# rrahn/libspm

Measured on AMD Instinct MI355X. Metric: Gbases/s scanned, Myers k<=3 |P|=100, higher is better.
Workload: dtype u32

## Files before the change

include/spm_hip.h:

```cpp
#ifndef SPM_HIP_H
#define SPM_HIP_H

#include <stddef.h>
#include <stdint.h>

#ifdef __cplusplus
extern "C" {
#endif

typedef struct spm_ctx spm_ctx;
typedef struct spm_text spm_text;
typedef struct spm_patterns spm_patterns;
typedef struct spm_hits spm_hits;
typedef struct spm_jst spm_jst;
typedef struct spm_jst_hits spm_jst_hits;

enum spm_status {
    SPM_OK = 0,
    SPM_E_INVALID = -1,
    SPM_E_HIP = -2,
    SPM_E_NOMEM = -3,
    SPM_E_UNSUPPORTED = -4,
    SPM_E_OVERFLOW = -5,
    SPM_E_PEER = -6
// ... 77 lines not shown
uint32_t spm_hip_patterns_count(const spm_patterns *p);
int spm_hip_patterns_needle(const spm_patterns *p, uint32_t pattern, uint8_t *out, uint32_t cap, uint32_t *len);

typedef struct spm_build_stats {
    float ms_total;
    float ms_tables;
    float ms_index;
    float ms_upload;
    uint32_t threads;
    uint32_t passes;
    uint32_t dense;
    uint32_t anchor_sixteenths;
    uint64_t keys;
    uint32_t stride, key_len;
    uint64_t bytes_device;
} spm_build_stats;
int spm_hip_patterns_build_stats(const spm_patterns *p, spm_build_stats *out);

size_t spm_hip_patterns_state_stride(const spm_patterns *p);
int spm_hip_patterns_state_init(const spm_patterns *p, void *state);

int spm_hip_scan(spm_ctx *ctx, const spm_text *text, uint64_t begin, uint64_t end, const spm_patterns *patterns,
                 const spm_scan_opts *opts, const void *state_in, void *state_out, spm_hits **out);

int spm_hip_scan_segments(spm_ctx *ctx, const spm_text *text, const uint64_t *seg_offsets, uint64_t n_segments,
                          const spm_patterns *patterns, const spm_scan_opts *opts, spm_hits **out);

int spm_hip_hits_view(spm_hits *hits, const spm_hit **records, uint64_t *n);
int spm_hip_hits_device(spm_hits *hits, const void **device_records, uint64_t *n);
int spm_hip_hits_copy_device(spm_hits *hits, void *device_dst, uint64_t cap, uint64_t *n);
// ... 668 lines not shown
```

libspm_amd/capi.py:

```python
from __future__ import annotations

import ctypes as C
import os
import subprocess

_PKG = os.path.dirname(os.path.abspath(__file__))
SO_PATH = os.path.join(_PKG, "libspm_hip.so")
CSRC = os.path.join(_PKG, "csrc")

ALGO_SHIFTOR, ALGO_MYERS, ALGO_MYERS_PREFIX, ALGO_HORSPOOL = 0, 1, 2, 3
ENGINE_AUTO, ENGINE_BRUTE, ENGINE_FILTER = 0, 1, 2
SCAN_IGNORE_PACKED = 1
SCAN_DEFER = 2
SCAN_ALIGNABLE = 4
MAX_NEEDLE = 2048


class SpmError(RuntimeError):
    pass


class Hit(C.Structure):
    _fields_ = [("pos", C.c_uint64), ("pattern", C.c_uint32), ("score", C.c_int32)]

# ... 28 lines not shown

class BuildStats(C.Structure):
    _fields_ = [
        ("ms_total", C.c_float),
        ("ms_tables", C.c_float),
        ("ms_index", C.c_float),
        ("ms_upload", C.c_float),
        ("threads", C.c_uint32),
        ("passes", C.c_uint32),
        ("dense", C.c_uint32),
        ("anchor_sixteenths", C.c_uint32),
        ("keys", C.c_uint64),
        ("stride", C.c_uint32),
        ("key_len", C.c_uint32),
        ("bytes_device", C.c_uint64),
    ]


class JstAllele(C.Structure):
    _fields_ = [("pos", C.c_uint64), ("ref_len", C.c_uint32), ("alt_len", C.c_uint32), ("alt_off", C.c_uint64)]


class JstHit(C.Structure):
    _fields_ = [("pos", C.c_uint64), ("haplotype", C.c_uint32), ("pattern", C.c_uint32), ("score", C.c_int32),
                ("reserved", C.c_uint32)]


class JstStats(C.Structure):
    _fields_ = [
        ("haplotype_symbols", C.c_uint64),
# ... 593 lines not shown
```

libspm_amd/csrc/filter_dense.hip:

```cpp
#include "filter_launch.hpp"
#include "filter_dense.hpp"

filter_kernel select_dense_kernel(const filter_index &F, bool km)
{
    if (F.dense) {
        switch (F.n_pat) {
        case 0:
        case 1: return seed_filter_dense_kernel<4, 1>;
        case 2: return seed_filter_dense_kernel<4, 2>;
        case 3: return seed_filter_dense_kernel<4, 3>;
        default: return nullptr;
        }
    }
    if (F.hash_variant == 4) {
        if (F.stride == 1)
            return km ? seed_filter_dense_kernel<4, 1, 1, true> : seed_filter_dense_kernel<4, 1, 1, false>;
        if (F.stride == 2)
            return km ? seed_filter_dense_kernel<4, 1, 2, true> : seed_filter_dense_kernel<4, 1, 2, false>;
    }
    return nullptr;
}

void warm_dense_kernels()
{
// ... 4 lines not shown
```

libspm_amd/csrc/filter_dense.hpp:

```cpp
#pragma once

#include "filter_stream.hpp"

namespace spm_hip
{

constexpr uint32_t kDenseQueueCap = 192;
constexpr int kDenseBatches = 3;

template <int NP>
__device__ __forceinline__ uint32_t dense_select(const filter_params &P, uint32_t w, uint32_t prev)
{
    const uint32_t X = alignbit(w, prev, 2);
    const uint32_t Y = alignbit(w, prev, 4);
    uint32_t sel = 0;
#pragma unroll
    for (int i = 0; i < NP; ++i) {
        const uint32_t C0 = (P.pat_c[i] & 3u) * 0x55555555u, M0 = (P.pat_cm[i] & 3u) * 0x55555555u;
        const uint32_t C1 = (P.pat_c[i] >> 2) * 0x55555555u, M1 = (P.pat_cm[i] >> 2) * 0x55555555u;
        uint32_t t = ((X ^ C0) & M0) | ((Y ^ C1) & M1);
        t |= t >> 1;
        sel |= ~t;
    }
    return sel & 0x55555555u;
}

struct dense_queue
{
    uint32_t key[kDenseQueueCap];
    uint32_t off[kDenseQueueCap];
};
static_assert(sizeof(dense_queue) == kDenseQueueBytes, "filter_params.hpp sizes the launch's LDS");

__device__ __forceinline__ void dense_drain(const filter_params &P, dense_queue &Q, uint32_t &qn, bool all, uint64_t span_base,
                                            uint32_t lane, const uint32_t *lds)
{
    while (qn >= 64 || (all && qn != 0)) {
// ... 25 lines not shown
            const uint32_t x0 = bk[b].x ^ f2, x1 = bk[b].y ^ f2, x2 = bk[b].z ^ f2, x3 = bk[b].w ^ f2;
            const uint32_t z = ((x0 - 0x00010001u) & ~x0) | ((x1 - 0x00010001u) & ~x1) | ((x2 - 0x00010001u) & ~x2) |
                               ((x3 - 0x00010001u) & ~x3);
            const bool hit = v[b] && ((z & 0x80008000u) != 0 || (bk[b].w >> 16) == kDenseAcceptAll);
            if (__ballot(hit) != 0) {
                if (__builtin_amdgcn_readfirstlane(cand_chunk_of(P, lds)[5]) == 0) {
                    const int64_t ts = (int64_t)span_base + (int64_t)off[b] - 16;
                    const bool has = hit && ts >= (int64_t)P.lo && (uint64_t)ts + P.key_len <= P.hi;
                    emit_survivors(P, has, key[b], has ? (uint64_t)ts : 0, lane, lds);
                }
            }
        }
    }
}

template <int UU, int NP, int S, bool KM>
__device__ __forceinline__ void dense_group(const filter_params &P, const uint4 (&cur)[UU], uint64_t gbase, uint64_t span_base,
                                            uint32_t &carry_in, uint32_t lane, const uint32_t *lds, dense_queue &Q, uint32_t &qn)
{
    static_assert(UU % 2 == 0 || UU == 1, "words are taken in pairs");
    uint32_t w[UU], prev[UU];
#pragma unroll
    for (int u = 0; u < UU; ++u)
        pack_with_prev(cur[u], lane, carry_in, w[u], prev[u]);
    const uint32_t goff = (uint32_t)(gbase - span_base) + lane * 16;
#pragma unroll
    for (int j = 0; j < UU; j += 2) {
        constexpr bool pair = UU > 1;
        const uint32_t w0 = w[j], p0 = prev[j], w1 = w[pair ? j + 1 : j], p1 = prev[pair ? j + 1 : j];
        const uint32_t kmask = KM ? P.key_mask : 0xFFFFFFFFu;
        static_assert(kDenseBloomBits == 20, "the word address below takes bits 5..19 of the index");
        uint32_t pm = 0;
        if constexpr (S == 0) {
            uint32_t todo = dense_select<NP>(P, w0, p0);
            if (pair)
                todo |= dense_select<NP>(P, w1, p1) << 1;
            while (todo != 0) {
                const uint32_t b = (uint32_t)__ffs(todo) - 1u;
                todo &= todo - 1;
                const bool odd = (b & 1u) != 0;
                const uint64_t both = ((uint64_t)(odd ? w1 : w0) << 32) | (odd ? p1 : p0);
                const uint32_t key = (uint32_t)(both >> ((b & ~1u) + 2u));
                const uint32_t h = key ^ (key >> 13);
                const uint32_t word = *reinterpret_cast<const uint32_t *>(reinterpret_cast<const uint8_t *>(lds) + ((h >> 3) & 0x1FFFCu));
                pm |= __builtin_amdgcn_ubfe(word, h, 1) << b;
            }
        } else {
#pragma unroll
            for (int u = 0; u < (pair ? 2 : 1); ++u) {
#pragma unroll
                for (int d = S; d <= 16; d += S) {
// ... 14 lines not shown
            const uint32_t key = (uint32_t)(both >> ((b & ~1u) + 2u)) & kmask;
            const uint64_t mm = __ballot(pos);
            if (pos) {
                const uint32_t q = qn + __popcll(mm & ((1ull << lane) - 1));
                Q.key[q] = key;
                Q.off[q] = goff + (uint32_t)j * 1024u + (odd ? 1024u : 0u) + (b >> 1) + 1u;
            }
            qn += __popcll(mm);
            queue_sync();
            if (qn > kDenseQueueCap - 64)
                dense_drain(P, Q, qn, false, span_base, lane, lds);
        }
    }
}

template <int U, int NP, int S = 0, bool KM = false>
__global__ __launch_bounds__(1024) void seed_filter_dense_kernel(const filter_params P)
{
    extern __shared__ uint32_t lds[];
    stream_stage(P, lds);

    const uint32_t lane = threadIdx.x & 63;
    const uint32_t waves_per_wg = blockDim.x >> 6;
    const uint32_t wave_in_wg = (uint32_t)__builtin_amdgcn_readfirstlane(threadIdx.x >> 6);
    dense_queue &Q = *reinterpret_cast<dense_queue *>(lds + P.lds_words + kCandLdsSlot + kCandRec * 16 +
                                                      (sizeof(dense_queue) / 4) * wave_in_wg);
    uint32_t qn = 0;

    const stream_geometry G = stream_geometry_of(P.lo, P.hi, 1024, P.span_chunks);
    const uint64_t span = P.span_chunks;
    const uint8_t *lane_text = P.text + G.base0 + (uint64_t)lane * 16;
// ... 18 lines not shown
#pragma unroll
            for (int u = 0; u < U; ++u)
                nxt[u] = load16_stream(lane_text + (ch + u) * 1024);
            for (; ch < fast_end; ch += U) {
                uint4 cur[U];
#pragma unroll
                for (int u = 0; u < U; ++u)
                    cur[u] = nxt[u];
                const bool more = ch + U < fast_end;
                const uint64_t pf = more ? ch + U : ch;
                const uint64_t ustride = more ? 1024 : 0;
#pragma unroll
                for (int u = 0; u < U; ++u)
                    nxt[u] = load16_stream(lane_text + pf * 1024 + (uint64_t)u * ustride);
                __builtin_amdgcn_sched_barrier(0);
                dense_group<U, NP, S, KM>(P, cur, G.base0 + ch * 1024, span_base, carry_in, lane, lds, Q, qn);
            }
        }
        for (; ch < c_end; ++ch) {
            uint4 one[1];
            one[0] = load_text16(P.text, G.base0 + ch * 1024 + (uint64_t)lane * 16, P.hi);
            dense_group<1, NP, S, KM>(P, one, G.base0 + ch * 1024, span_base, carry_in, lane, lds, Q, qn);
        }
        dense_drain(P, Q, qn, true, span_base, lane, lds);
    }
    surv_close(P, cand_chunk_of(P, lds), lane);
}

}
```

libspm_amd/csrc/filter_shared.hpp:

```cpp
#pragma once

#include "hd.hpp"

namespace spm_hip
{

constexpr uint32_t kKeyMax = 16;
constexpr uint32_t kKeyMin = 9;
constexpr double kMaxSurvivorShare = 0.08;

constexpr uint32_t kMergeMinK = 8;
struct seed_plan
{
    uint32_t n, q;
};
SPM_HD inline seed_plan plan_seeds(uint32_t m, uint32_t k)
{
    const uint32_t surplus = (k >= kMergeMinK && k <= 1000 && m / (k + 2) >= kKeyMin) ? 2u : 1u;
    return {k + surplus, m / (k + surplus)};
}

constexpr uint32_t kBloomProbes = 4;

SPM_HD inline uint32_t bloom_hash(uint32_t key, uint32_t i)
// ... 34 lines not shown
    return x ^ (x >> 16);
}

constexpr uint32_t kDensePatterns = 3;
constexpr uint32_t kDenseBloomBits = 20;
constexpr uint32_t kDenseSlots = 8;
constexpr uint32_t kDenseAcceptAll = 0x7FFFu;

SPM_HD inline uint32_t dense_bloom_index(uint32_t key)
{
    return (key ^ (key >> 13)) & ((1u << kDenseBloomBits) - 1);
}
SPM_HD inline uint32_t dense_bucket(uint32_t key, uint32_t bucket_shift) { return (key * 0x9E3779B1u) >> bucket_shift; }
SPM_HD inline uint32_t dense_fp(uint32_t key) { return 0x8000u | ((key ^ (key >> 15) ^ (key >> 23)) & 0x7FFFu); }

SPM_HD inline bool dense_anchored(uint32_t d, const uint32_t *c, const uint32_t *cm, uint32_t n_pat)
{
    for (uint32_t i = 0; i < n_pat; ++i)
        if (((d ^ c[i]) & cm[i]) == 0)
            return true;
    return false;
}

constexpr uint32_t kRngRun = 0x8000u;
constexpr uint32_t kRngSingle = 0x2000u;
constexpr uint32_t kRngWhole = 0x1000u;
constexpr uint32_t kSeedChecked = 0x4000u;

}
```

libspm_amd/csrc/index_dense.hpp:

```cpp
#pragma once

#include <chrono>
#include <cstdio>

#include "index_tables.hpp"

namespace spm_hip
{

struct dense_anchor_set
{
    uint32_t n_pat = 0, c[kDensePatterns] = {0, 0, 0}, cm[kDensePatterns] = {0, 0, 0};
    uint32_t dimers = 0;
    uint32_t sixteenths() const { return (uint32_t)__builtin_popcount(dimers); }
};

inline dense_anchor_set anchor_union(const dense_anchor_set &a, uint32_t c, uint32_t cm)
{
    dense_anchor_set r = a;
    r.c[r.n_pat] = c & cm;
    r.cm[r.n_pat] = cm;
    ++r.n_pat;
    r.dimers |= dimer_mask_of(c, cm);
    return r;
}

inline uint32_t dense_pick(const uint8_t *pat, uint32_t m, uint32_t dimers, uint32_t c, uint32_t want, uint16_t *pos)
{
    if (m < kKeyMax)
        return 0;
    uint32_t n = 0;
    for (uint32_t i = 0; i + kKeyMax <= m && n < want; ++i) {
        if (!((dimers >> dimer_at(pat, i)) & 1u))
            continue;
        if (n >= c && i < (uint32_t)pos[n - c] + kKeyMax)
            continue;
        pos[n++] = (uint16_t)i;
    }
    return n;
}

constexpr uint32_t kDenseCmax = 4;

inline uint32_t dense_layout(const uint8_t *pat, uint32_t m, uint32_t k, uint32_t dimers, uint16_t *pos, uint32_t &n_out)
{
    for (uint32_t c = 1; c <= kDenseCmax; ++c) {
        const uint32_t want = c * k + 1;
        if (want > 255)
            break;
        if (dense_pick(pat, m, dimers, c, want, pos) == want) {
            n_out = want;
            return c;
        }
    }
    return 0;
}

constexpr uint32_t kDenseMaxPieces = kDenseCmax * 7 + 1;

inline bool dense_eligible(const needle_view &nv)
{
    if (nv.sigma != 4 || nv.max_k >= kMergeMinK || nv.n == 0)
        return false;
    for (uint32_t p = 0; p < nv.n; ++p) {
        const uint32_t m = (uint32_t)nv.m[p];
        if (m < kKeyMax * (nv.errors(p) + 1) || m > 2047)
            return false;
    }
    return true;
}

inline uint64_t dense_uncovered(const needle_view &nv, uint32_t dimers, size_t begin, size_t end, size_t step,
                                std::vector<uint32_t> *list = nullptr, size_t cap = 0)
{
    uint64_t bad = 0;
    uint16_t pos[kDenseMaxPieces];
    for (size_t p = begin; p < end; p += step) {
        uint32_t n = 0;
        if (dense_layout(nv.needle(p), (uint32_t)nv.m[p], nv.errors(p), dimers, pos, n) == 0) {
            ++bad;
            if (list && list->size() < cap)
                list->push_back((uint32_t)p);
        }
    }
    return bad;
}

struct anchor_search
{
    const needle_view &nv;
    unsigned nt;
    size_t sample_step;
    std::vector<uint32_t> hard;
};

inline uint64_t uncovered_all(anchor_search &S, uint32_t dimers)
{
    std::vector<uint64_t> part(S.nt, 0);
    std::vector<std::vector<uint32_t>> lists(S.nt);
    parallel_slices(S.nv.n, S.nt,
                    [&](size_t b, size_t e, unsigned t) { part[t] = dense_uncovered(S.nv, dimers, b, e, 1, &lists[t], 8); });
    uint64_t s = 0;
    for (unsigned t = 0; t < S.nt; ++t) {
        s += part[t];
        for (uint32_t p : lists[t])
            if (S.hard.size() < 256)
                S.hard.push_back(p);
    }
    return s;
}

inline bool try_rung(anchor_search &S, const std::vector<dense_anchor_set> &cands, dense_anchor_set &best_seen)
{
    const needle_view &nv = S.nv;
    std::vector<uint64_t> base(cands.size(), 0);
    parallel_slices(cands.size(), S.nt, [&](size_t b, size_t e, unsigned) {
        for (size_t i = b; i < e; ++i)
            base[i] = dense_uncovered(nv, cands[i].dimers, 0, nv.n, S.sample_step);
    });
    std::vector<uint8_t> tried(cands.size(), 0);
    uint64_t best_fail = ~0ull;
    for (int attempt = 0; attempt < 4; ++attempt) {
        size_t best = cands.size();
        uint64_t best_bad = ~0ull;
        for (size_t i = 0; i < cands.size(); ++i) {
            if (tried[i])
                continue;
            uint64_t bad = base[i];
            for (uint32_t p : S.hard)
                bad += 4096 * dense_uncovered(nv, cands[i].dimers, p, (size_t)p + 1, 1);
            if (bad < best_bad) {
                best_bad = bad;
                best = i;
            }
        }
        if (best == cands.size())
            break;
        tried[best] = 1;
        const size_t hard_before = S.hard.size();
        const uint64_t fail = uncovered_all(S, cands[best].dimers);
        if (fail < best_fail) {
            best_fail = fail;
            best_seen = cands[best];
        }
        if (fail == 0)
            return true;
        if (S.hard.size() == hard_before || fail > nv.n / 2000 + 4)
            break;
        uint64_t placed = 0, asked = 0;
        for (size_t h = hard_before; h < S.hard.size(); ++h)
            for (size_t i = 0; i < cands.size(); i += 3) {
                ++asked;
                placed += dense_uncovered(nv, cands[i].dimers, S.hard[h], (size_t)S.hard[h] + 1, 1) == 0 ? 1 : 0;
            }
        if (2 * placed > asked)
            break;
    }
    return false;
}

inline std::vector<dense_anchor_set> anchor_extensions(const dense_anchor_set &base, uint32_t care)
{
    std::vector<dense_anchor_set> r;
    for (uint32_t cm = 0; cm < 16; ++cm) {
        if ((uint32_t)__builtin_popcount(cm) != care)
            continue;
        for (uint32_t c = 0; c < 16; ++c)
            if ((c & ~cm) == 0 && (dimer_mask_of(c, cm) & base.dimers) == 0)
                r.push_back(anchor_union(base, c, cm));
    }
    return r;
}

struct anchor_rung
{
    int extends;
    uint32_t care;
    bool dimer_pairs;
};
constexpr anchor_rung kAnchorLadder[] = {
    {-1, 3, true},
    {0, 4, false},
    {-1, 2, false},
    {2, 4, false},
    {2, 3, false},
    {-1, 1, false},
    {5, 2, false},
    {-1, 0, false},
};
constexpr size_t kAnchorRungs = sizeof(kAnchorLadder) / sizeof(kAnchorLadder[0]);

inline std::vector<dense_anchor_set> rung_candidates(const anchor_rung &R, const dense_anchor_set *best_of_rung)
{
    const dense_anchor_set none;
    std::vector<dense_anchor_set> c = anchor_extensions(R.extends < 0 ? none : best_of_rung[R.extends], R.care);
    if (R.dimer_pairs)
        for (uint32_t d0 = 0; d0 < 16; ++d0)
            for (uint32_t d1 = d0 + 1; d1 < 16; ++d1)
                if (__builtin_popcount(d0 ^ d1) != 1)
                    c.push_back(anchor_union(anchor_union(none, d0, 15), d1, 15));
    return c;
}

inline bool choose_dense_anchors(const needle_view &nv, const index_tuning &T, dense_anchor_set &out)
{
    anchor_search S{nv, T.n_threads(), std::max<size_t>(1, nv.n / 1024), {}};
    const int max_density = T.dense >= 2 ? 16 : 8;
    dense_anchor_set best_of_rung[kAnchorRungs];
    for (size_t rung = 0; rung < kAnchorRungs; ++rung) {
        const std::vector<dense_anchor_set> c = rung_candidates(kAnchorLadder[rung], best_of_rung);
        if (c.empty() || (int)c[0].sixteenths() < T.dense_min_density)
            continue;
        if ((int)c[0].sixteenths() > max_density)
            return false;
        if (try_rung(S, c, best_of_rung[rung])) {
            out = best_of_rung[rung];
            return true;
        }
    }
    return false;
}

struct dense_layouts
{
    std::vector<uint8_t> c, n;
    std::vector<uint32_t> first;
    std::vector<uint16_t> pos;
};

inline dense_layouts dense_first_fit(const needle_view &nv, unsigned nt, uint32_t dimers)
{
    dense_layouts L;
    L.c.assign(nv.n, 0);
    L.n.assign(nv.n, 0);
    L.first.assign(nv.n + 1, 0);
    std::vector<std::vector<uint16_t>> pos_of(nt);
    parallel_slices(nv.n, nt, [&](size_t b, size_t e, unsigned t) {
        uint16_t pos[kDenseMaxPieces];
        std::vector<uint16_t> &out = pos_of[t];
        out.reserve((e - b) * 5);
        for (size_t p = b; p < e; ++p) {
            uint32_t n = 0;
            L.c[p] = (uint8_t)dense_layout(nv.needle(p), (uint32_t)nv.m[p], nv.errors(p), dimers, pos, n);
            L.n[p] = (uint8_t)n;
            out.insert(out.end(), pos, pos + n);
        }
    });
    for (uint32_t p = 0; p < nv.n; ++p)
        L.first[p + 1] = L.first[p] + L.n[p];
    L.pos.reserve(L.first[nv.n]);
    for (unsigned t = 0; t < nt; ++t)
        L.pos.insert(L.pos.end(), pos_of[t].begin(), pos_of[t].end());
    return L;
}

inline void dense_share_bits(const needle_view &nv, const index_tuning &T, uint32_t dimers, const std::vector<uint8_t> &cc,
                             const std::vector<uint32_t> &first, std::vector<uint16_t> &pos_flat)
{
    thread_team team(T.n_threads());
    std::vector<uint16_t> ref(1u << kDenseBloomBits, 0);
    std::vector<uint8_t> placed(nv.n, 0);
    std::vector<uint32_t> bit_of(pos_flat.size(), 0), fresh_bit(pos_flat.size(), 0);
    for (uint32_t p = 0; p < nv.n; ++p)
        if (cc[p] != 1) {
            for (uint32_t s = first[p]; s < first[p + 1]; ++s)
                ++ref[bit_of[s] = dense_bloom_index(window_key(4, nv.needle(p), pos_flat[s], kKeyMax))];
            placed[p] = 1;
        }
    constexpr uint32_t kRounds = 24;
    std::vector<uint16_t> fresh(pos_flat.size());
    const unsigned nt = team.size();
// ... 14 lines not shown
                    const uint32_t need = first[p + 1] - first[p];
                    if (cc[p] != 1 || need == 0)
                        continue;
                    const uint8_t *pat = nv.needle(p);
                    const uint32_t m = (uint32_t)nv.m[p];
                    uint32_t own[kDenseMaxPieces];
                    for (uint32_t j = 0; j < need; ++j)
                        own[j] = placed[p] ? bit_of[first[p] + j] : 0xFFFFFFFFu;
                    cpos.clear();
                    cbit.clear();
                    shared.clear();
                    uint32_t key = window_key(4, pat, 0, kKeyMax);
                    for (uint32_t i = 0; i + kKeyMax <= m; ++i) {
                        if (i)
                            key = (key >> 2) | ((uint32_t)(pat[i + kKeyMax - 1] & 3u) << 30);
                        if (!((dimers >> (key & 15u)) & 1u))
                            continue;
                        const uint32_t bit = dense_bloom_index(key);
                        uint32_t mine = 0;
                        for (uint32_t j = 0; j < need; ++j)
                            mine += own[j] == bit ? 1u : 0u;
                        cpos.push_back((uint16_t)i);
                        cbit.push_back(bit);
                        shared.push_back(ref[bit] > mine ? 1 : 0);
                    }
                    const uint32_t nc = (uint32_t)cpos.size();
                    nxt.assign(nc + 1, nc);
                    for (uint32_t i = 0, t = 0; i < nc; ++i) {
                        while (t < nc && cpos[t] < cpos[i] + kKeyMax)
                            ++t;
                        nxt[i] = t;
// ... 84 lines not shown
    });
    return keys;
}

inline filter_index dense_pass_header(const dense_anchor_set &A, size_t n_keys)
{
    filter_index F;
    F.dense = 1;
    F.key_len = kKeyMax;
    F.stride = 1;
    F.n_pat = A.n_pat;
    for (uint32_t i = 0; i < A.n_pat; ++i) {
        F.pat_c[i] = A.c[i];
        F.pat_cm[i] = A.cm[i];
    }
    F.dimer_set = A.dimers;
    F.n_keys = n_keys;
    F.n_entries = n_keys;
    F.hash_variant = 3;
    return F;
}

inline int build_dense_index(const needle_view &nv, const index_tuning &T, seed_index &X)
{
    using iclk = std::chrono::steady_clock;
    auto ms = [&](iclk::time_point a) { return std::chrono::duration<double, std::milli>(iclk::now() - a).count(); };
    const unsigned nt = T.n_threads();
    const auto t0 = iclk::now();
    dense_anchor_set A;
    if (!choose_dense_anchors(nv, T, A))
        return SPM_OK;
    const double ms_anchors = ms(t0);
    const auto t1 = iclk::now();
    dense_layouts L = dense_first_fit(nv, nt, A.dimers);
    const double ms_first_fit = ms(t1);
    dense_share_bits(nv, T, A.dimers, L.c, L.first, L.pos);
    const double ms_share = ms(t1) - ms_first_fit;
    std::vector<index_kv> keys = dense_pieces(nv, nt, L, X);
    const double ms_layout = ms(t1);
    const auto t2 = iclk::now();
    filter_index F = dense_pass_header(A, keys.size());
    build_bits_level1(keys, F);
    const double ms_level1 = ms(t2);
    const auto t3 = iclk::now();
    build_directory(keys, F, X.h_entries);
    if (trace_on()) {
        uint64_t set = 0;
        for (uint32_t w : F.h_image)
            set += (uint64_t)__builtin_popcount(w);
        fprintf(stderr, "[spm_hip] dense index: %zu keys, anchors %u/16 (%u pattern(s)), %.1f %% of the presence bits set; anchors %.2f ms, "
                        "layouts %.2f (first fit %.2f, shared bits %.2f), bits + buckets %.2f, directory %.2f (%u threads)\n",
                keys.size(), A.sixteenths(), A.n_pat, 100.0 * (double)set / (double)(1u << kDenseBloomBits), ms_anchors, ms_layout,
                ms_first_fit, ms_share, ms_level1, ms(t3), nt);
    }
    F.ok = true;
    X.fidx.push_back(std::move(F));
    X.filter_stride = 1;
    X.filter_key_len = kKeyMax;
    X.filter_anchored = false;
    X.filter_dense = true;
    X.filter_max_range = 0;
    return SPM_OK;
}

}
```

libspm_amd/csrc/index_selftest.hpp:

```cpp
#pragma once

#include <cstring>

namespace spm_hip
{

inline bool level1_accepts(const filter_index &F, uint32_t key)
{
    if (F.dense || F.hash_variant == 4) {
        if (F.dense && !((F.dimer_set >> (key & 15u)) & 1u))
            return false;
        const uint32_t b = dense_bloom_index(key);
        if (!((F.h_image[b >> 5] >> (b & 31)) & 1u))
            return false;
        const uint16_t *bk = F.h_buckets.data() + (size_t)dense_bucket(key, F.bucket_shift) * kDenseSlots;
        if (bk[kDenseSlots - 1] == kDenseAcceptAll)
            return true;
        for (uint32_t s = 0; s < kDenseSlots; ++s)
            if (bk[s] == dense_fp(key))
                return true;
        return false;
    }
    if (F.hash_variant == 2) {
        const uint16_t *fp = reinterpret_cast<const uint16_t *>(F.h_image.data());
        const uint16_t *disp = reinterpret_cast<const uint16_t *>(reinterpret_cast<const uint8_t *>(F.h_image.data()) + F.chd_disp_off);
// ... 66 lines not shown
            if (q < kKeyMax || o + q > m)
                return SPM_E_INVALID;
            for (uint32_t i = 0; i < q; ++i)
                if (++cover[o + i] > c)
                    return SPM_E_INVALID;
            uint32_t found = 0;
            for (uint32_t r = 0; r + kKeyMax <= q; ++r)
                found += window_indexed(nv, X, F, p, o + r) ? 1 : 0;
            ++checked;
            missing += found < 1 ? 1 : 0;
        }
    }
    stats[3] = checked;
    stats[4] = missing;
    selftest_false_positives(F, stats);
    stats[7] = 3u | ((uint64_t)__builtin_popcount(F.dimer_set & 0xFFFFu) << 8) | (deep << 16);
    return missing ? SPM_E_INVALID : SPM_OK;
}

inline bool selftest_seeds_sound(const needle_view &nv, const seed_index &X, uint32_t p)
{
    const uint32_t q = X.seed_q[p], sn = X.seed_n[p];
    if (X.filter_stride > q - (X.filter_key_len - 1) || sn < (uint32_t)nv.k[p] + 1)
        return false;
    for (uint32_t j = 0; j < sn; ++j) {
        const uint32_t o = X.seed_off[X.seed_first[p] + j];
        if (o + q > (uint32_t)nv.m[p] || (j && o < (uint32_t)X.seed_off[X.seed_first[p] + j - 1] + q))
            return false;
        for (uint32_t i = 0; i < q; ++i)
            if (!key_symbol(nv.sigma, nv.needle(p)[o + i]))
                return false;
// ... 110 lines not shown
```

libspm_amd/csrc/index_types.hpp:

```cpp
#pragma once

#include <algorithm>
#include <cstdint>
#include <thread>
#include <utility>
#include <vector>

#include "../../include/spm_hip.h"
#include "filter_shared.hpp"
#include "host_util.hpp"

namespace spm_hip
{

struct index_tuning
{
    int force_stride = 0;
    int max_keys = 57344;
    int hash = 2;
    int anchor = 1;
    int dedupe = 1;
    int dense = 1;
    int dense_min_density = 0;
    int threads = 0;
    static index_tuning from_env()
    {
        index_tuning T;
        T.force_stride = env_int("SPM_HIP_FILTER_STRIDE", 0);
        T.max_keys = std::max(1024, env_int("SPM_HIP_FILTER_MAX_KEYS", 57344));
        T.hash = std::max(1, std::min(2, env_int("SPM_HIP_FILTER_HASH", 2)));
        T.anchor = env_int("SPM_HIP_FILTER_ANCHOR", 1);
        T.dedupe = env_int("SPM_HIP_FILTER_DEDUPE", 1);
        T.dense = env_int("SPM_HIP_FILTER_DENSE", 1);
        T.dense_min_density = env_int("SPM_HIP_FILTER_DENSE_MIN_DENSITY", 0);
        T.threads = env_int("SPM_HIP_BUILD_THREADS", 0);
        return T;
    }
    unsigned n_threads() const
    {
        if (threads > 0)
            return (unsigned)std::min(threads, 64);
        const unsigned hc = std::thread::hardware_concurrency();
        return std::max(1u, std::min(16u, hc ? hc : 1u));
    }
};

struct needle_view
{
    int algo = 0;
    uint32_t n = 0, sigma = 4;
// ... 1 lines not shown
    const uint32_t *offsets = nullptr;
    const int32_t *m = nullptr, *k = nullptr;
    uint32_t max_k = 0;
    bool is_myers() const { return algo == SPM_ALGO_MYERS || algo == SPM_ALGO_MYERS_PREFIX; }
    const uint8_t *needle(size_t p) const { return ranks + offsets[p]; }
    uint32_t errors(size_t p) const { return is_myers() ? (uint32_t)k[p] : 0; }
};

struct filter_index
{
    uint32_t anchor_c = 0, anchor_cm = 0;
    bool ok = false;
    uint32_t dense = 0;
    uint32_t n_pat = 0, pat_c[kDensePatterns] = {0, 0, 0}, pat_cm[kDensePatterns] = {0, 0, 0};
    uint32_t dimer_set = 0xFFFF;
    uint32_t bucket_shift = 0;
    uint32_t stride = 0;
    uint32_t key_len = 16;
    uint32_t bitmap_words = 0;
    uint32_t n_probes = 0;
    uint32_t hash_variant = 0;
    uint32_t lds_words = 0;
    uint32_t chd_slot_mask = 0, chd_bucket_shift = 0, chd_disp_off = 0;
    uint32_t ht_mask = 0;
    uint64_t n_keys = 0;
    uint64_t n_entries = 0;
    uint32_t max_range = 0;
    std::vector<uint32_t> h_image;
    std::vector<u32x4> h_ht;
    std::vector<uint16_t> h_buckets;
// ... 37 lines not shown
    for (uint32_t i = 0; i < H; ++i)
        key |= key_code(sigma, pat[at + i]) << (2 * i);
    return key;
}

inline uint32_t dimer_at(const uint8_t *pat, uint32_t at) { return (pat[at] & 3u) | ((uint32_t)(pat[at + 1] & 3u) << 2); }

inline uint32_t dimer_mask_of(uint32_t c, uint32_t cm)
{
    uint32_t set = 0;
    for (uint32_t d = 0; d < 16; ++d)
        set |= (((d ^ c) & cm) == 0 ? 1u : 0u) << d;
    return set;
}

inline bool layout_seeds(const needle_view &nv, uint32_t p, uint32_t q_floor, uint32_t &n_out, uint32_t &q_out,
                         std::vector<uint16_t> &off)
{
    const uint32_t m = (uint32_t)nv.m[p], k = nv.errors(p);
    const uint8_t *pat = nv.needle(p);
    bool clean = true;
    for (uint32_t i = 0; i < m; ++i)
        clean = clean && key_symbol(nv.sigma, pat[i]);
    const seed_plan sp = plan_seeds(m, k);
    off.clear();
    if (clean) {
        n_out = sp.n;
        q_out = sp.q;
        for (uint32_t j = 0; j < sp.n; ++j)
            off.push_back((uint16_t)(j * sp.q));
// ... 55 lines not shown
```

libspm_amd/csrc/patterns.hip:

```cpp
#include "internal.hpp"
#include "index_build.hpp"
#include "strands.hpp"
#include "tables_build.hpp"

namespace
{
struct needle_upload
{
    struct item
    {
        void **dst;
        const void *src;
        size_t bytes, off;
    };
    std::vector<item> items;
    size_t total = 0;
    size_t add(void **dst, const void *src, size_t bytes, size_t zero_tail = 0)
    {
        items.push_back(item{dst, src, bytes, total});
        total += (std::max<size_t>(bytes + zero_tail, 16) + 255) & ~(size_t)255;
        return items.size() - 1;
    }
    hipError_t place(void **arena)
    {
// ... 127 lines not shown
    }

    if ((sigma == 4 || sigma == 5 || sigma == 15) && algo != SPM_ALGO_MYERS_PREFIX && n_patterns > 0) {
        const auto ti = clk::now();
        int rc = build_filter_index(nv, tune, *ps);
        if (rc != SPM_OK)
            return rc;
        ps->build.ms_index = ms_since(ti);
        if (!ps->fidx.empty()) {
            for (filter_index &F : ps->fidx) {
                SPM_HIP_CHECK(ctx, upload(&F.d_bitmap, F.h_image.data(), F.h_image.size() * sizeof(uint32_t)));
                SPM_HIP_CHECK(ctx, upload(&F.d_ht, F.h_ht.data(), F.h_ht.size() * sizeof(u32x4)));
                if (!F.h_buckets.empty())
                    SPM_HIP_CHECK(ctx, upload(&F.d_buckets, F.h_buckets.data(), F.h_buckets.size() * sizeof(uint16_t)));
                ps->build.keys += F.n_keys;
                for (uint32_t d = 0; d < 16; ++d)
                    ps->build.anchor_sixteenths += (F.dimer_set >> d) & 1u;
            }
            pass_tab_item = (long)up.add(reinterpret_cast<void **>(&ps->d_pass_tab), nullptr, ps->fidx.size() * sizeof(pass_entry));
            SPM_HIP_CHECK(ctx, upload(&ps->d_entries, ps->h_entries.data(), ps->h_entries.size() * sizeof(u32x4)));
            up.add(reinterpret_cast<void **>(&ps->d_ranks), ps->ranks.data(), ps->ranks.size(), 64);
            SPM_HIP_CHECK(ctx, upload(&ps->d_offsets, ps->offsets.data(), ps->offsets.size() * sizeof(uint32_t)));
            if (ps->sigma == 4) {
                pack_needles(nv, pk, pk_off, tune.n_threads());
                SPM_HIP_CHECK(ctx, upload(&ps->d_needle_pk, pk.data(), pk.size() * sizeof(uint32_t)));
                SPM_HIP_CHECK(ctx, upload(&ps->d_pk_offsets, pk_off.data(), pk_off.size() * sizeof(uint32_t)));
            }
            SPM_HIP_CHECK(ctx, upload(&ps->d_seed_q, ps->seed_q.data(), ps->seed_q.size() * sizeof(uint16_t)));
        }
        if (!ps->fidx.empty() && ps->max_k >= kMergeMinK && ps->max_k <= 1000) {
            surplus.assign(ps->m.size(), 1);
            for (uint32_t p = 0; p < ps->n; ++p)
// ... 18 lines not shown
        }
        ps->h_entries = std::vector<u32x4>();
        ps->build.bytes_device = up.total;
        ms_upload = ms_since(tu);
        if (spm_trace_on())
            fprintf(stderr, "[spm_hip] patterns_create: one allocation of %.2f MiB in %.2f ms, streamed up in %.2f ms\n",
                    up.total / 1048576.0, ms_place, ms_upload - ms_place);
    }
    ps->build.ms_upload = (float)ms_upload;
    ps->build.ms_total = ms_since(t_begin);
    ps->build.passes = (uint32_t)ps->fidx.size();
    ps->build.dense = ps->filter_dense ? 1u : 0u;
    ps->build.stride = ps->filter_stride;
    ps->build.key_len = ps->filter_key_len;
    if (spm_trace_on())
        fprintf(stderr, "[spm_hip] patterns_create: %u needles, algo %d, sigma %u -> %u pass(es)%s, %llu keys, %u/16 of the dimers; "
                        "%.2f ms (tables %.2f, index %.2f, upload %.2f; %u threads)\n",
                n_patterns, algo, sigma, ps->build.passes, ps->build.dense ? " dense" : "", (unsigned long long)ps->build.keys,
                ps->build.anchor_sixteenths, ps->build.ms_total, ps->build.ms_tables, ps->build.ms_index, ps->build.ms_upload,
                ps->build.threads);
    *out = ps.release();
    return SPM_OK;
}

extern "C" int spm_hip_patterns_create_stranded(spm_ctx *ctx, int algo, const uint8_t *ranks_concat, const uint32_t *offsets,
                                                uint32_t n_reads, const uint16_t *k, uint32_t sigma, spm_patterns **out)
{
    if (!ctx || !out || (n_reads && (!offsets || !ranks_concat)) || sigma < 2 || sigma > 255 || algo < 0 ||
        algo > SPM_ALGO_HORSPOOL) {
        SPM_SET_ERR(ctx, "spm_hip_patterns_create_stranded: invalid argument");
        return SPM_E_INVALID;
    }
    const stranded_set S = build_stranded(ranks_concat, offsets, n_reads, k, sigma);
    if (S.status != SPM_OK) {
// ... 195 lines not shown
```

Measured before the change: 6509.

## Extend dense filter anchors from dimers to trimers for sparser candidate selection

The dense seed filter now chooses anchor patterns over 3-symbol windows (64 classes) instead of 2-symbol windows (16 classes). The anchor search ladder gains trimer rungs that refine a nearly-covering dimer set, and the kernel gets a T3 variant that also compares a third shifted symbol. The aim is to select fewer text positions for bloom and bucket probes per scanned base. In exchange it adds index-build search cost and a few extra ALU ops per word in the select step.

```diff
diff --git a/include/spm_hip.h b/include/spm_hip.h
--- a/include/spm_hip.h
+++ b/include/spm_hip.h
@@ -115,6 +115,8 @@
     uint64_t keys;
     uint32_t stride, key_len;
     uint64_t bytes_device;
+    uint32_t anchor_64ths;
+    uint32_t reserved;
 } spm_build_stats;
 int spm_hip_patterns_build_stats(const spm_patterns *p, spm_build_stats *out);
 
diff --git a/libspm_amd/capi.py b/libspm_amd/capi.py
--- a/libspm_amd/capi.py
+++ b/libspm_amd/capi.py
@@ -66,6 +66,8 @@
         ("stride", C.c_uint32),
         ("key_len", C.c_uint32),
         ("bytes_device", C.c_uint64),
+        ("anchor_64ths", C.c_uint32),
+        ("reserved", C.c_uint32),
     ]
 
 
diff --git a/libspm_amd/csrc/filter_dense.hip b/libspm_amd/csrc/filter_dense.hip
--- a/libspm_amd/csrc/filter_dense.hip
+++ b/libspm_amd/csrc/filter_dense.hip
@@ -4,6 +4,12 @@
 filter_kernel select_dense_kernel(const filter_index &F, bool km)
 {
     if (F.dense) {
+        if (dense_third_symbol(F.pat_cm, F.n_pat))
+            switch (F.n_pat) {
+            case 2: return seed_filter_dense_kernel<4, 2, 0, false, true>;
+            case 3: return seed_filter_dense_kernel<4, 3, 0, false, true>;
+            default: return nullptr;
+            }
         switch (F.n_pat) {
         case 0:
         case 1: return seed_filter_dense_kernel<4, 1>;
diff --git a/libspm_amd/csrc/filter_dense.hpp b/libspm_amd/csrc/filter_dense.hpp
--- a/libspm_amd/csrc/filter_dense.hpp
+++ b/libspm_amd/csrc/filter_dense.hpp
@@ -8,19 +8,32 @@
 constexpr uint32_t kDenseQueueCap = 192;
 constexpr int kDenseBatches = 3;
 
-template <int NP>
+template <int NP, bool T3>
 __device__ __forceinline__ uint32_t dense_select(const filter_params &P, uint32_t w, uint32_t prev)
 {
     const uint32_t X = alignbit(w, prev, 2);
     const uint32_t Y = alignbit(w, prev, 4);
     uint32_t sel = 0;
-#pragma unroll
-    for (int i = 0; i < NP; ++i) {
-        const uint32_t C0 = (P.pat_c[i] & 3u) * 0x55555555u, M0 = (P.pat_cm[i] & 3u) * 0x55555555u;
-        const uint32_t C1 = (P.pat_c[i] >> 2) * 0x55555555u, M1 = (P.pat_cm[i] >> 2) * 0x55555555u;
-        uint32_t t = ((X ^ C0) & M0) | ((Y ^ C1) & M1);
-        t |= t >> 1;
-        sel |= ~t;
+    if constexpr (T3) {
+        const uint32_t Z = alignbit(w, prev, 6);
+#pragma unroll
+        for (int i = 0; i < NP; ++i) {
+            const uint32_t C0 = (P.pat_c[i] & 3u) * 0x55555555u, M0 = (P.pat_cm[i] & 3u) * 0x55555555u;
+            const uint32_t C1 = ((P.pat_c[i] >> 2) & 3u) * 0x55555555u, M1 = ((P.pat_cm[i] >> 2) & 3u) * 0x55555555u;
+            const uint32_t C2 = (P.pat_c[i] >> 4) * 0x55555555u, M2 = (P.pat_cm[i] >> 4) * 0x55555555u;
+            uint32_t t = ((X ^ C0) & M0) | ((Y ^ C1) & M1) | ((Z ^ C2) & M2);
+            t |= t >> 1;
+            sel |= ~t;
+        }
+    } else {
+#pragma unroll
+        for (int i = 0; i < NP; ++i) {
+            const uint32_t C0 = (P.pat_c[i] & 3u) * 0x55555555u, M0 = (P.pat_cm[i] & 3u) * 0x55555555u;
+            const uint32_t C1 = (P.pat_c[i] >> 2) * 0x55555555u, M1 = (P.pat_cm[i] >> 2) * 0x55555555u;
+            uint32_t t = ((X ^ C0) & M0) | ((Y ^ C1) & M1);
+            t |= t >> 1;
+            sel |= ~t;
+        }
     }
     return sel & 0x55555555u;
 }
@@ -76,7 +89,7 @@
     }
 }
 
-template <int UU, int NP, int S, bool KM>
+template <int UU, int NP, int S, bool KM, bool T3>
 __device__ __forceinline__ void dense_group(const filter_params &P, const uint4 (&cur)[UU], uint64_t gbase, uint64_t span_base,
                                             uint32_t &carry_in, uint32_t lane, const uint32_t *lds, dense_queue &Q, uint32_t &qn)
 {
@@ -94,9 +107,9 @@
         static_assert(kDenseBloomBits == 20, "the word address below takes bits 5..19 of the index");
         uint32_t pm = 0;
         if constexpr (S == 0) {
-            uint32_t todo = dense_select<NP>(P, w0, p0);
+            uint32_t todo = dense_select<NP, T3>(P, w0, p0);
             if (pair)
-                todo |= dense_select<NP>(P, w1, p1) << 1;
+                todo |= dense_select<NP, T3>(P, w1, p1) << 1;
             while (todo != 0) {
                 const uint32_t b = (uint32_t)__ffs(todo) - 1u;
                 todo &= todo - 1;
@@ -141,7 +154,7 @@
     }
 }
 
-template <int U, int NP, int S = 0, bool KM = false>
+template <int U, int NP, int S = 0, bool KM = false, bool T3 = false>
 __global__ __launch_bounds__(1024) void seed_filter_dense_kernel(const filter_params P)
 {
     extern __shared__ uint32_t lds[];
@@ -190,13 +203,13 @@
                 for (int u = 0; u < U; ++u)
                     nxt[u] = load16_stream(lane_text + pf * 1024 + (uint64_t)u * ustride);
                 __builtin_amdgcn_sched_barrier(0);
-                dense_group<U, NP, S, KM>(P, cur, G.base0 + ch * 1024, span_base, carry_in, lane, lds, Q, qn);
+                dense_group<U, NP, S, KM, T3>(P, cur, G.base0 + ch * 1024, span_base, carry_in, lane, lds, Q, qn);
             }
         }
         for (; ch < c_end; ++ch) {
             uint4 one[1];
             one[0] = load_text16(P.text, G.base0 + ch * 1024 + (uint64_t)lane * 16, P.hi);
-            dense_group<1, NP, S, KM>(P, one, G.base0 + ch * 1024, span_base, carry_in, lane, lds, Q, qn);
+            dense_group<1, NP, S, KM, T3>(P, one, G.base0 + ch * 1024, span_base, carry_in, lane, lds, Q, qn);
         }
         dense_drain(P, Q, qn, true, span_base, lane, lds);
     }
diff --git a/libspm_amd/csrc/filter_shared.hpp b/libspm_amd/csrc/filter_shared.hpp
--- a/libspm_amd/csrc/filter_shared.hpp
+++ b/libspm_amd/csrc/filter_shared.hpp
@@ -72,12 +72,19 @@
 SPM_HD inline uint32_t dense_bucket(uint32_t key, uint32_t bucket_shift) { return (key * 0x9E3779B1u) >> bucket_shift; }
 SPM_HD inline uint32_t dense_fp(uint32_t key) { return 0x8000u | ((key ^ (key >> 15) ^ (key >> 23)) & 0x7FFFu); }
 
-SPM_HD inline bool dense_anchored(uint32_t d, const uint32_t *c, const uint32_t *cm, uint32_t n_pat)
+SPM_HD inline bool dense_anchored(uint32_t t, const uint32_t *c, const uint32_t *cm, uint32_t n_pat)
 {
     for (uint32_t i = 0; i < n_pat; ++i)
-        if (((d ^ c[i]) & cm[i]) == 0)
+        if (((t ^ c[i]) & cm[i]) == 0)
             return true;
     return false;
+}
+SPM_HD inline bool dense_third_symbol(const uint32_t *cm, uint32_t n_pat)
+{
+    uint32_t any = 0;
+    for (uint32_t i = 0; i < n_pat; ++i)
+        any |= cm[i] >> 4;
+    return any != 0;
 }
 
 constexpr uint32_t kRngRun = 0x8000u;
diff --git a/libspm_amd/csrc/index_dense.hpp b/libspm_amd/csrc/index_dense.hpp
--- a/libspm_amd/csrc/index_dense.hpp
+++ b/libspm_amd/csrc/index_dense.hpp
@@ -11,8 +11,8 @@
 struct dense_anchor_set
 {
     uint32_t n_pat = 0, c[kDensePatterns] = {0, 0, 0}, cm[kDensePatterns] = {0, 0, 0};
-    uint32_t dimers = 0;
-    uint32_t sixteenths() const { return (uint32_t)__builtin_popcount(dimers); }
+    uint64_t trimers = 0;
+    uint32_t sixty_fourths() const { return (uint32_t)__builtin_popcountll(trimers); }
 };
 
 inline dense_anchor_set anchor_union(const dense_anchor_set &a, uint32_t c, uint32_t cm)
@@ -21,17 +21,17 @@
     r.c[r.n_pat] = c & cm;
     r.cm[r.n_pat] = cm;
     ++r.n_pat;
-    r.dimers |= dimer_mask_of(c, cm);
+    r.trimers |= trimer_mask_of(c, cm);
     return r;
 }
 
-inline uint32_t dense_pick(const uint8_t *pat, uint32_t m, uint32_t dimers, uint32_t c, uint32_t want, uint16_t *pos)
+inline uint32_t dense_pick(const uint8_t *pat, uint32_t m, uint64_t trimers, uint32_t c, uint32_t want, uint16_t *pos)
 {
     if (m < kKeyMax)
         return 0;
     uint32_t n = 0;
     for (uint32_t i = 0; i + kKeyMax <= m && n < want; ++i) {
-        if (!((dimers >> dimer_at(pat, i)) & 1u))
+        if (!((trimers >> trimer_at(pat, i)) & 1u))
             continue;
         if (n >= c && i < (uint32_t)pos[n - c] + kKeyMax)
             continue;
@@ -42,13 +42,13 @@
 
 constexpr uint32_t kDenseCmax = 4;
 
-inline uint32_t dense_layout(const uint8_t *pat, uint32_t m, uint32_t k, uint32_t dimers, uint16_t *pos, uint32_t &n_out)
+inline uint32_t dense_layout(const uint8_t *pat, uint32_t m, uint32_t k, uint64_t trimers, uint16_t *pos, uint32_t &n_out)
 {
     for (uint32_t c = 1; c <= kDenseCmax; ++c) {
         const uint32_t want = c * k + 1;
         if (want > 255)
             break;
-        if (dense_pick(pat, m, dimers, c, want, pos) == want) {
+        if (dense_pick(pat, m, trimers, c, want, pos) == want) {
             n_out = want;
             return c;
         }
@@ -70,14 +70,14 @@
     return true;
 }
 
-inline uint64_t dense_uncovered(const needle_view &nv, uint32_t dimers, size_t begin, size_t end, size_t step,
+inline uint64_t dense_uncovered(const needle_view &nv, uint64_t trimers, size_t begin, size_t end, size_t step,
                                 std::vector<uint32_t> *list = nullptr, size_t cap = 0)
 {
     uint64_t bad = 0;
     uint16_t pos[kDenseMaxPieces];
     for (size_t p = begin; p < end; p += step) {
         uint32_t n = 0;
-        if (dense_layout(nv.needle(p), (uint32_t)nv.m[p], nv.errors(p), dimers, pos, n) == 0) {
+        if (dense_layout(nv.needle(p), (uint32_t)nv.m[p], nv.errors(p), trimers, pos, n) == 0) {
             ++bad;
             if (list && list->size() < cap)
                 list->push_back((uint32_t)p);
@@ -92,34 +92,45 @@
     unsigned nt;
     size_t sample_step;
     std::vector<uint32_t> hard;
+    size_t close() const { return nv.n / 256 + 8; }
 };
 
-inline uint64_t uncovered_all(anchor_search &S, uint32_t dimers)
+struct rung_result
+{
+    uint64_t fail = ~0ull;
+    std::vector<uint32_t> failed;
+};
+
+inline uint64_t uncovered_all(anchor_search &S, uint64_t trimers, std::vector<uint32_t> &failed)
 {
     std::vector<uint64_t> part(S.nt, 0);
     std::vector<std::vector<uint32_t>> lists(S.nt);
-    parallel_slices(S.nv.n, S.nt,
-                    [&](size_t b, size_t e, unsigned t) { part[t] = dense_uncovered(S.nv, dimers, b, e, 1, &lists[t], 8); });
+    parallel_slices(S.nv.n, S.nt, [&](size_t b, size_t e, unsigned t) {
+        part[t] = dense_uncovered(S.nv, trimers, b, e, 1, &lists[t], std::max<size_t>(8, S.close()));
+    });
     uint64_t s = 0;
+    failed.clear();
     for (unsigned t = 0; t < S.nt; ++t) {
         s += part[t];
-        for (uint32_t p : lists[t])
-            if (S.hard.size() < 256)
-                S.hard.push_back(p);
+        for (size_t i = 0; i < lists[t].size(); ++i) {
+            if (i < 8 && S.hard.size() < 256)
+                S.hard.push_back(lists[t][i]);
+            failed.push_back(lists[t][i]);
+        }
     }
     return s;
 }
 
-inline bool try_rung(anchor_search &S, const std::vector<dense_anchor_set> &cands, dense_anchor_set &best_seen)
+inline bool try_rung(anchor_search &S, const std::vector<dense_anchor_set> &cands, dense_anchor_set &best_seen, rung_result &left)
 {
     const needle_view &nv = S.nv;
     std::vector<uint64_t> base(cands.size(), 0);
     parallel_slices(cands.size(), S.nt, [&](size_t b, size_t e, unsigned) {
         for (size_t i = b; i < e; ++i)
-            base[i] = dense_uncovered(nv, cands[i].dimers, 0, nv.n, S.sample_step);
+            base[i] = dense_uncovered(nv, cands[i].trimers, 0, nv.n, S.sample_step);
     });
     std::vector<uint8_t> tried(cands.size(), 0);
-    uint64_t best_fail = ~0ull;
+    std::vector<uint32_t> failed;
     for (int attempt = 0; attempt < 4; ++attempt) {
         size_t best = cands.size();
         uint64_t best_bad = ~0ull;
@@ -128,7 +139,7 @@
                 continue;
             uint64_t bad = base[i];
             for (uint32_t p : S.hard)
-                bad += 4096 * dense_uncovered(nv, cands[i].dimers, p, (size_t)p + 1, 1);
+                bad += 4096 * dense_uncovered(nv, cands[i].trimers, p, (size_t)p + 1, 1);
             if (bad < best_bad) {
                 best_bad = bad;
                 best = i;
@@ -138,9 +149,10 @@
             break;
         tried[best] = 1;
         const size_t hard_before = S.hard.size();
-        const uint64_t fail = uncovered_all(S, cands[best].dimers);
-        if (fail < best_fail) {
-            best_fail = fail;
+        const uint64_t fail = uncovered_all(S, cands[best].trimers, failed);
+        if (fail < left.fail) {
+            left.fail = fail;
+            left.failed.swap(failed);
             best_seen = cands[best];
         }
         if (fail == 0)
@@ -151,7 +163,7 @@
         for (size_t h = hard_before; h < S.hard.size(); ++h)
             for (size_t i = 0; i < cands.size(); i += 3) {
                 ++asked;
-                placed += dense_uncovered(nv, cands[i].dimers, S.hard[h], (size_t)S.hard[h] + 1, 1) == 0 ? 1 : 0;
+                placed += dense_uncovered(nv, cands[i].trimers, S.hard[h], (size_t)S.hard[h] + 1, 1) == 0 ? 1 : 0;
             }
         if (2 * placed > asked)
             break;
@@ -159,14 +171,37 @@
     return false;
 }
 
-inline std::vector<dense_anchor_set> anchor_extensions(const dense_anchor_set &base, uint32_t care)
+inline bool try_trimer_rung(anchor_search &S, const std::vector<dense_anchor_set> &cands, const rung_result &below,
+                            dense_anchor_set &best_seen)
+{
+    if (below.fail > S.close() || below.failed.size() != below.fail)
+        return false;
+    std::vector<uint64_t> bad(cands.size(), 0);
+    parallel_slices(cands.size(), S.nt, [&](size_t b, size_t e, unsigned) {
+        for (size_t i = b; i < e; ++i)
+            for (uint32_t p : below.failed)
+                bad[i] += dense_uncovered(S.nv, cands[i].trimers, p, (size_t)p + 1, 1);
+    });
+    const size_t best = (size_t)(std::min_element(bad.begin(), bad.end()) - bad.begin());
+    best_seen = cands[best];
+    if (bad[best] != 0)
+        return false;
+    std::vector<uint32_t> hard_before = S.hard, failed;
+    const uint64_t fail = uncovered_all(S, cands[best].trimers, failed);
+    S.hard.swap(hard_before);
+    return fail == 0;
+}
+
+inline std::vector<dense_anchor_set> anchor_extensions(const dense_anchor_set &base, uint32_t care, uint32_t bits)
 {
     std::vector<dense_anchor_set> r;
-    for (uint32_t cm = 0; cm < 16; ++cm) {
+    if (base.n_pat >= kDensePatterns)
+        return r;
+    for (uint32_t cm = 0; cm < (1u << bits); ++cm) {
         if ((uint32_t)__builtin_popcount(cm) != care)
             continue;
-        for (uint32_t c = 0; c < 16; ++c)
-            if ((c & ~cm) == 0 && (dimer_mask_of(c, cm) & base.dimers) == 0)
+        for (uint32_t c = 0; c < (1u << bits); ++c)
+            if ((c & ~cm) == 0 && (trimer_mask_of(c, cm) & base.trimers) == 0)
                 r.push_back(anchor_union(base, c, cm));
     }
     return r;
@@ -176,24 +211,29 @@
 {
     int extends;
     uint32_t care;
+    bool trimer;
     bool dimer_pairs;
 };
 constexpr anchor_rung kAnchorLadder[] = {
-    {-1, 3, true},
-    {0, 4, false},
-    {-1, 2, false},
-    {2, 4, false},
-    {2, 3, false},
-    {-1, 1, false},
-    {5, 2, false},
-    {-1, 0, false},
+    {-1, 3, false, true},
+    {0, 5, true, false},
+    {0, 4, false, false},
+    {2, 5, true, false},
+    {-1, 2, false, false},
+    {4, 5, true, false},
+    {4, 4, false, false},
+    {6, 5, true, false},
+    {4, 3, false, false},
+    {-1, 1, false, false},
+    {9, 2, false, false},
+    {-1, 0, false, false},
 };
 constexpr size_t kAnchorRungs = sizeof(kAnchorLadder) / sizeof(kAnchorLadder[0]);
 
 inline std::vector<dense_anchor_set> rung_candidates(const anchor_rung &R, const dense_anchor_set *best_of_rung)
 {
     const dense_anchor_set none;
-    std::vector<dense_anchor_set> c = anchor_extensions(R.extends < 0 ? none : best_of_rung[R.extends], R.care);
+    std::vector<dense_anchor_set> c = anchor_extensions(R.extends < 0 ? none : best_of_rung[R.extends], R.care, R.trimer ? 6 : 4);
     if (R.dimer_pairs)
         for (uint32_t d0 = 0; d0 < 16; ++d0)
             for (uint32_t d1 = d0 + 1; d1 < 16; ++d1)
@@ -205,15 +245,19 @@
 inline bool choose_dense_anchors(const needle_view &nv, const index_tuning &T, dense_anchor_set &out)
 {
     anchor_search S{nv, T.n_threads(), std::max<size_t>(1, nv.n / 1024), {}};
-    const int max_density = T.dense >= 2 ? 16 : 8;
+    const int max_density = T.dense >= 2 ? 64 : 32;
     dense_anchor_set best_of_rung[kAnchorRungs];
+    rung_result left[kAnchorRungs];
     for (size_t rung = 0; rung < kAnchorRungs; ++rung) {
-        const std::vector<dense_anchor_set> c = rung_candidates(kAnchorLadder[rung], best_of_rung);
-        if (c.empty() || (int)c[0].sixteenths() < T.dense_min_density)
+        const anchor_rung &R = kAnchorLadder[rung];
+        if (R.trimer && (!T.dense_trimers || left[R.extends].fail > S.close()))
             continue;
-        if ((int)c[0].sixteenths() > max_density)
+        const std::vector<dense_anchor_set> c = rung_candidates(R, best_of_rung);
+        if (c.empty() || (int)c[0].sixty_fourths() < 4 * T.dense_min_density)
+            continue;
+        if ((int)c[0].sixty_fourths() > max_density)
             return false;
-        if (try_rung(S, c, best_of_rung[rung])) {
+        if (R.trimer ? try_trimer_rung(S, c, left[R.extends], best_of_rung[rung]) : try_rung(S, c, best_of_rung[rung], left[rung])) {
             out = best_of_rung[rung];
             return true;
         }
@@ -228,7 +272,7 @@
     std::vector<uint16_t> pos;
 };
 
-inline dense_layouts dense_first_fit(const needle_view &nv, unsigned nt, uint32_t dimers)
+inline dense_layouts dense_first_fit(const needle_view &nv, unsigned nt, uint64_t trimers)
 {
     dense_layouts L;
     L.c.assign(nv.n, 0);
@@ -241,7 +285,7 @@
         out.reserve((e - b) * 5);
         for (size_t p = b; p < e; ++p) {
             uint32_t n = 0;
-            L.c[p] = (uint8_t)dense_layout(nv.needle(p), (uint32_t)nv.m[p], nv.errors(p), dimers, pos, n);
+            L.c[p] = (uint8_t)dense_layout(nv.needle(p), (uint32_t)nv.m[p], nv.errors(p), trimers, pos, n);
             L.n[p] = (uint8_t)n;
             out.insert(out.end(), pos, pos + n);
         }
@@ -254,7 +298,7 @@
     return L;
 }
 
-inline void dense_share_bits(const needle_view &nv, const index_tuning &T, uint32_t dimers, const std::vector<uint8_t> &cc,
+inline void dense_share_bits(const needle_view &nv, const index_tuning &T, uint64_t trimers, const std::vector<uint8_t> &cc,
                              const std::vector<uint32_t> &first, std::vector<uint16_t> &pos_flat)
 {
     thread_team team(T.n_threads());
@@ -299,7 +343,7 @@
                     for (uint32_t i = 0; i + kKeyMax <= m; ++i) {
                         if (i)
                             key = (key >> 2) | ((uint32_t)(pat[i + kKeyMax - 1] & 3u) << 30);
-                        if (!((dimers >> (key & 15u)) & 1u))
+                        if (!((trimers >> (key & 63u)) & 1u))
                             continue;
                         const uint32_t bit = dense_bloom_index(key);
                         uint32_t mine = 0;
@@ -414,7 +458,8 @@
         F.pat_c[i] = A.c[i];
         F.pat_cm[i] = A.cm[i];
     }
-    F.dimer_set = A.dimers;
+    F.trimer_set = A.trimers;
+    F.dimer_set = dimers_of_trimers(A.trimers);
     F.n_keys = n_keys;
     F.n_entries = n_keys;
     F.hash_variant = 3;
@@ -432,9 +477,9 @@
         return SPM_OK;
     const double ms_anchors = ms(t0);
     const auto t1 = iclk::now();
-    dense_layouts L = dense_first_fit(nv, nt, A.dimers);
+    dense_layouts L = dense_first_fit(nv, nt, A.trimers);
     const double ms_first_fit = ms(t1);
-    dense_share_bits(nv, T, A.dimers, L.c, L.first, L.pos);
+    dense_share_bits(nv, T, A.trimers, L.c, L.first, L.pos);
     const double ms_share = ms(t1) - ms_first_fit;
     std::vector<index_kv> keys = dense_pieces(nv, nt, L, X);
     const double ms_layout = ms(t1);
@@ -448,9 +493,9 @@
         uint64_t set = 0;
         for (uint32_t w : F.h_image)
             set += (uint64_t)__builtin_popcount(w);
-        fprintf(stderr, "[spm_hip] dense index: %zu keys, anchors %u/16 (%u pattern(s)), %.1f %% of the presence bits set; anchors %.2f ms, "
+        fprintf(stderr, "[spm_hip] dense index: %zu keys, anchors %u/64 (%u pattern(s)), %.1f %% of the presence bits set; anchors %.2f ms, "
                         "layouts %.2f (first fit %.2f, shared bits %.2f), bits + buckets %.2f, directory %.2f (%u threads)\n",
-                keys.size(), A.sixteenths(), A.n_pat, 100.0 * (double)set / (double)(1u << kDenseBloomBits), ms_anchors, ms_layout,
+                keys.size(), A.sixty_fourths(), A.n_pat, 100.0 * (double)set / (double)(1u << kDenseBloomBits), ms_anchors, ms_layout,
                 ms_first_fit, ms_share, ms_level1, ms(t3), nt);
     }
     F.ok = true;
diff --git a/libspm_amd/csrc/index_selftest.hpp b/libspm_amd/csrc/index_selftest.hpp
--- a/libspm_amd/csrc/index_selftest.hpp
+++ b/libspm_amd/csrc/index_selftest.hpp
@@ -8,7 +8,7 @@
 inline bool level1_accepts(const filter_index &F, uint32_t key)
 {
     if (F.dense || F.hash_variant == 4) {
-        if (F.dense && !((F.dimer_set >> (key & 15u)) & 1u))
+        if (F.dense && !((F.trimer_set >> (key & 63u)) & 1u))
             return false;
         const uint32_t b = dense_bloom_index(key);
         if (!((F.h_image[b >> 5] >> (b & 31)) & 1u))
@@ -105,7 +105,7 @@
     stats[3] = checked;
     stats[4] = missing;
     selftest_false_positives(F, stats);
-    stats[7] = 3u | ((uint64_t)__builtin_popcount(F.dimer_set & 0xFFFFu) << 8) | (deep << 16);
+    stats[7] = 3u | ((uint64_t)((F.anchored_64ths() + 3) / 4) << 8) | (deep << 16);
     return missing ? SPM_E_INVALID : SPM_OK;
 }
 
diff --git a/libspm_amd/csrc/index_types.hpp b/libspm_amd/csrc/index_types.hpp
--- a/libspm_amd/csrc/index_types.hpp
+++ b/libspm_amd/csrc/index_types.hpp
@@ -22,6 +22,7 @@
     int dedupe = 1;
     int dense = 1;
     int dense_min_density = 0;
+    int dense_trimers = 0;
     int threads = 0;
     static index_tuning from_env()
     {
@@ -34,6 +35,7 @@
         T.dense = env_int("SPM_HIP_FILTER_DENSE", 1);
         T.dense_min_density = env_int("SPM_HIP_FILTER_DENSE_MIN_DENSITY", 0);
         T.threads = env_int("SPM_HIP_BUILD_THREADS", 0);
+        T.dense_trimers = 1;
         return T;
     }
     unsigned n_threads() const
@@ -65,6 +67,11 @@
     uint32_t dense = 0;
     uint32_t n_pat = 0, pat_c[kDensePatterns] = {0, 0, 0}, pat_cm[kDensePatterns] = {0, 0, 0};
     uint32_t dimer_set = 0xFFFF;
+    uint64_t trimer_set = ~0ull;
+    uint32_t anchored_64ths() const
+    {
+        return dense ? (uint32_t)__builtin_popcountll(trimer_set) : 4u * (uint32_t)__builtin_popcount(dimer_set & 0xFFFFu);
+    }
     uint32_t bucket_shift = 0;
     uint32_t stride = 0;
     uint32_t key_len = 16;
@@ -132,6 +139,22 @@
     return set;
 }
 
+inline uint32_t trimer_at(const uint8_t *pat, uint32_t at) { return dimer_at(pat, at) | ((uint32_t)(pat[at + 2] & 3u) << 4); }
+
+inline uint64_t trimer_mask_of(uint32_t c, uint32_t cm)
+{
+    uint64_t set = 0;
+    for (uint32_t t = 0; t < 64; ++t)
+        set |= (uint64_t)(((t ^ c) & cm) == 0 ? 1u : 0u) << t;
+    return set;
+}
+
+inline uint32_t dimers_of_trimers(uint64_t trimers)
+{
+    const uint64_t any = trimers | (trimers >> 16) | (trimers >> 32) | (trimers >> 48);
+    return (uint32_t)(any & 0xFFFFu);
+}
+
 inline bool layout_seeds(const needle_view &nv, uint32_t p, uint32_t q_floor, uint32_t &n_out, uint32_t &q_out,
                          std::vector<uint16_t> &off)
 {
diff --git a/libspm_amd/csrc/patterns.hip b/libspm_amd/csrc/patterns.hip
--- a/libspm_amd/csrc/patterns.hip
+++ b/libspm_amd/csrc/patterns.hip
@@ -165,8 +165,8 @@
                 if (!F.h_buckets.empty())
                     SPM_HIP_CHECK(ctx, upload(&F.d_buckets, F.h_buckets.data(), F.h_buckets.size() * sizeof(uint16_t)));
                 ps->build.keys += F.n_keys;
-                for (uint32_t d = 0; d < 16; ++d)
-                    ps->build.anchor_sixteenths += (F.dimer_set >> d) & 1u;
+                ps->build.anchor_64ths += F.anchored_64ths();
+                ps->build.anchor_sixteenths += (F.anchored_64ths() + 3) / 4;
             }
             pass_tab_item = (long)up.add(reinterpret_cast<void **>(&ps->d_pass_tab), nullptr, ps->fidx.size() * sizeof(pass_entry));
             SPM_HIP_CHECK(ctx, upload(&ps->d_entries, ps->h_entries.data(), ps->h_entries.size() * sizeof(u32x4)));
@@ -215,10 +215,10 @@
     ps->build.stride = ps->filter_stride;
     ps->build.key_len = ps->filter_key_len;
     if (spm_trace_on())
-        fprintf(stderr, "[spm_hip] patterns_create: %u needles, algo %d, sigma %u -> %u pass(es)%s, %llu keys, %u/16 of the dimers; "
+        fprintf(stderr, "[spm_hip] patterns_create: %u needles, algo %d, sigma %u -> %u pass(es)%s, %llu keys, %u/16 of the windows (%u/64); "
                         "%.2f ms (tables %.2f, index %.2f, upload %.2f; %u threads)\n",
                 n_patterns, algo, sigma, ps->build.passes, ps->build.dense ? " dense" : "", (unsigned long long)ps->build.keys,
-                ps->build.anchor_sixteenths, ps->build.ms_total, ps->build.ms_tables, ps->build.ms_index, ps->build.ms_upload,
+                ps->build.anchor_sixteenths, ps->build.anchor_64ths, ps->build.ms_total, ps->build.ms_tables, ps->build.ms_index, ps->build.ms_upload,
                 ps->build.threads);
     *out = ps.release();
     return SPM_OK;
```

Result: no change. 6510 (median of 2 runs) (+0.0%).
